# maxwellsh/DIGDriver

Measured on AMD Instinct MI355X. Metric: genomic elements tested/sec (whole node), whole-genome x 37 cohorts, higher is better.
Workload: dtype f64

## Files before the change

digdriver_amd/csrc/dig_nb.hip:

```cpp
#include <algorithm>
#include <cstdlib>

#include "dig_common.hpp"
#include "dig_math.hpp"

namespace dig {

constexpr int kBlock = 256;

struct OpMidpUpper {
    __device__ static double apply(double k, double a, double p) { return nb_midp_upper(k, a, p); }
};
struct OpExact {
    __device__ static double apply(double k, double a, double p) { return nb_exact(k, a, p); }
};
struct OpGreater {
    __device__ static double apply(double k, double a, double p) { return nb_greater(k, a, p); }
};
struct OpMidpTwo {
    __device__ static double apply(double k, double a, double p) { return nb_midp_twosided(k, a, p); }
};

template <typename Op>
__global__ __launch_bounds__(kBlock) void nb3_kernel(const double* __restrict__ k, const double* __restrict__ alpha,
// ... 96 lines not shown
    const int64_t e = a.use_fastdiv ? fastdiv(i, a.divC) : i;
    return load_raw(a, i, e, i - e * a.C);
}

__device__ __forceinline__ PairInputs prepare_pair(const PairRaw& w, bool has_indel_params)
{
    PairInputs r;
    r.k_snv = (double)w.k_snv;
    r.k_smp = (double)w.k_smp;
    r.k_ind = (double)w.k_ind;
    const GammaParams g = normal_params_to_gamma(w.mu, w.sigma);
    r.alpha = g.alpha;
    r.theta = mul_rn(g.theta, w.cj);
    r.exp_snv = mul_rn(mul_rn(g.alpha, r.theta), w.pi_s);
    r.p = nb_success_prob(r.theta, w.pi_s);
    GammaParams gi = g;
    if (has_indel_params) gi = normal_params_to_gamma(w.mu_i, w.sigma_i);
    r.alpha_i = gi.alpha;
    r.theta_i = mul_rn(gi.theta, w.cji);
    r.exp_ind = mul_rn(mul_rn(gi.alpha, r.theta_i), w.pi_i);
    r.p_i = nb_success_prob(r.theta_i, w.pi_i);
    return r;
}

__device__ __forceinline__ PairInputs load_pair(const ElementStatsArgs& a, int64_t i)
{
    return prepare_pair(load_raw(a, i), a.mu_indel != nullptr);
}

__global__ __launch_bounds__(kBlock) void element_stats_single_pass_kernel(ElementStatsArgs a)
{
    nb_tables_init();
    const int64_t n = a.E * a.C;
    const int64_t i = (int64_t)blockIdx.x * kBlock + threadIdx.x;
    if (i >= n) return;
    const PairInputs q = load_pair(a, i);
    double pv_snv = 0.0, pv_smp = 0.0, pv_ind = 0.0, dummy = 0.0;
    const unsigned d1 = nb_midp_upper_fast2(q.k_snv, q.k_smp, 3u, q.alpha, q.p, pv_snv, pv_smp);
    const unsigned d2 = nb_midp_upper_fast2(q.k_ind, 0.0, 1u, q.alpha_i, q.p_i, pv_ind, dummy);
    if (!(d1 & 1u)) pv_snv = nb_midp_upper_unresolved(q.k_snv, q.alpha, q.p);
    if (!(d1 & 2u)) pv_smp = nb_midp_upper_unresolved(q.k_smp, q.alpha, q.p);
    if (!(d2 & 1u)) pv_ind = nb_midp_upper_unresolved(q.k_ind, q.alpha_i, q.p_i);
    a.out[0 * n + i] = q.exp_snv;
    a.out[1 * n + i] = pv_snv;
    a.out[2 * n + i] = pv_smp;
    a.out[3 * n + i] = q.theta_i;
    a.out[4 * n + i] = q.exp_ind;
    a.out[5 * n + i] = pv_ind;
    a.out[6 * n + i] = fisher_combine_fast(pv_snv, pv_ind);
}

constexpr int kParkCap = 256;

__device__ __forceinline__ unsigned park_flush(unsigned* worklist, const unsigned* park, unsigned count, int lane)
{
    unsigned base = 0;
    if (lane == 0) base = atomicAdd(worklist, count);
    base = __shfl(base, 0, 64);
    for (unsigned j = lane; j < count; j += 64) worklist[kWorkHeader + base + j] = park[j];
    return 0;
}

#define DIG_STREAM_STORE(ptr, val) __builtin_nontemporal_store((val), (ptr))
template <bool HAS_INDEL_PARAMS, bool FUSED_RATES = false>
__global__ __launch_bounds__(kBlock) void element_stats_stream_kernel(ElementStatsArgs a)
{
    static_assert(!FUSED_RATES, "the rate sums are formed by element_stats_stream_fused_kernel");
    __shared__ unsigned park_all[kBlock / 64][kParkCap];
    nb_tables_init();
    unsigned* park = park_all[threadIdx.x >> 6];
    const int64_t n = a.E * a.C;
    const int lane = threadIdx.x & 63;
    const unsigned long long lanes_below = (1ull << lane) - 1ull;
    const int64_t n_tiles = (n + 63) >> 6;
    const int64_t n_waves = ((int64_t)gridDim.x * kBlock) >> 6;
    int64_t tile = ((int64_t)blockIdx.x * kBlock + threadIdx.x) >> 6;
    if (tile >= n_tiles) return;
    const int64_t step_pairs = n_waves * 64;
    const int64_t step_e = a.use_fastdiv ? fastdiv(step_pairs, a.divC) : step_pairs;
    const uint32_t step_c = (uint32_t)(step_pairs - step_e * a.C);
    const uint32_t C32 = (uint32_t)a.C;
    int64_t iu = tile * 64 + lane;
    int64_t eu = a.use_fastdiv ? fastdiv(iu, a.divC) : iu;
    uint32_t cu = (uint32_t)(iu - eu * a.C);
    auto clamped_load = [&]() {
        const bool past = iu >= n;
        return load_raw(a, past ? n - 1 : iu, past ? a.E - 1 : eu, past ? (int64_t)(C32 - 1) : (int64_t)cu);
    };
    PairRaw nxt = clamped_load();
    unsigned parked = 0;
    for (; tile < n_tiles; tile += n_waves) {
        if (parked > (unsigned)(kParkCap - 64)) parked = park_flush(a.worklist, park, parked, lane);
        const int64_t i_raw = tile * 64 + lane;
        const int64_t i = min(i_raw, n - 1);
        PairRaw cur = nxt;
        iu += step_pairs;
        eu += step_e;
        cu += step_c;
        if (cu >= C32) {
            cu -= C32;
            eu += 1;
        }
        nxt = clamped_load();
        const PairInputs q = prepare_pair(cur, HAS_INDEL_PARAMS);
        double pv_snv, pv_smp, pv_ind, dummy;
        const unsigned d1 = nb_fast2_counts<1>(cur.k_snv, cur.k_smp, true, q.alpha, q.p, pv_snv, pv_smp);
        const unsigned d2 = nb_fast2_counts<1>(cur.k_ind, 0, false, q.alpha_i, q.p_i, pv_ind, dummy);
        const bool slow = ((d1 != 3u) || (d2 != 1u)) && i_raw < n;
        const unsigned long long m = __ballot(slow);
        if (slow) park[parked + __popcll(m & lanes_below)] = (unsigned)i;
        parked += (unsigned)__popcll(m);
        DIG_STREAM_STORE(&a.out[0 * n + i], q.exp_snv);
        DIG_STREAM_STORE(&a.out[1 * n + i], pv_snv);
        DIG_STREAM_STORE(&a.out[2 * n + i], pv_smp);
        DIG_STREAM_STORE(&a.out[3 * n + i], q.theta_i);
        DIG_STREAM_STORE(&a.out[4 * n + i], q.exp_ind);
        DIG_STREAM_STORE(&a.out[5 * n + i], pv_ind);
        double pv_mut = 0.0;
        if (!slow) pv_mut = fisher_combine_fast(pv_snv, pv_ind);
        DIG_STREAM_STORE(&a.out[6 * n + i], pv_mut);
    }
    if (parked) park_flush(a.worklist, park, parked, lane);
}

constexpr int kPre = 2;

struct StagePtr {
    int64_t q0, q1;
    uint32_t i, e, c;
    uint32_t ok;
};
struct StageIn {
    int32_t idx[kPre];
    double mu, sg, mu_i, sg_i;
    double pi_s, pi_i, cj, cji;
    int k_snv, k_smp, k_ind;
    int64_t q0;
    uint32_t nb, i, c;
};
struct StageBin {
    double mu[kPre], sd[kPre];
    int32_t y[kPre];
    uint8_t fl[kPre];
};

constexpr int kQueueCap = 1024;
constexpr int kRecDoubles = 11;
__shared__ double g_queue[kQueueCap * kRecDoubles];
typedef double v2d __attribute__((ext_vector_type(2)));
__shared__ unsigned g_queue_list[16][48];
__shared__ unsigned g_queue_len, g_ovf_len, g_ovf_next;
__shared__ unsigned g_tests[3 * kQueueCap];
__shared__ unsigned g_n_tests, g_next_test;
constexpr int kSlowBlock = 256;
constexpr int kSlowWaves = kSlowBlock / 64;
constexpr int kSlowPairsPerWave = 8;
constexpr int kOverflowSlack = 64 * 1024;
__device__ __forceinline__ void slow_round(const ElementStatsArgs& a, const unsigned* __restrict__ items, unsigned base,
                                           unsigned count, bool have_first, unsigned first_item, double (*sp_all)[10],
                                           unsigned* list, int64_t n);

template <int TB, bool TICKETS, int GIVEN = 0, bool REC = false>
__global__ __launch_bounds__(TB) void element_stats_stream_fused_kernel(ElementStatsArgs a)
{
    static_assert(TB == 1024 && TICKETS, "one 1024-thread workgroup per CU drawing tile tickets");
    static_assert(!REC || GIVEN == 0 || GIVEN == 3, "record outputs: the pipeline's kernel only");
    double* const queue = g_queue;
    unsigned* const tests = g_tests;
    constexpr int QCAP = kQueueCap;
    constexpr bool FUSED = GIVEN == 0 || GIVEN == 3;
    constexpr bool PACKED = GIVEN == 3;
    __shared__ unsigned park_all[TB / 64][kParkCap];
    __shared__ unsigned s_ticket;
    if (threadIdx.x == 0) s_ticket = 0;
    if (threadIdx.x == 0) g_queue_len = g_ovf_len = g_ovf_next = g_n_tests = g_next_test = 0;
    nb_tables_init();
    unsigned* park = park_all[threadIdx.x >> 6];
    const int64_t n = a.E * a.C;
    const int lane = threadIdx.x & 63;
    const unsigned long long lanes_below = (1ull << lane) - 1ull;
    const int64_t n_tiles = (n + 63) >> 6;
    int64_t tile = ((int64_t)blockIdx.x * TB + threadIdx.x) >> 6;
    const uint32_t C32 = (uint32_t)a.C;
    int64_t iu = tile * 64 + lane;
    int64_t eu = a.use_fastdiv ? fastdiv(iu, a.divC) : iu;
    uint32_t cu = (uint32_t)(iu - eu * a.C);
    auto draw = [&]() -> int64_t {
        unsigned t = 0;
        if (lane == 0) t = atomicAdd(&s_ticket, 1u);
        t = (unsigned)__builtin_amdgcn_readfirstlane((int)t);
        if ((gridDim.x & 7u) == 0u) return ((int64_t)t * 8 + (blockIdx.x & 7u)) * (gridDim.x >> 3) + (blockIdx.x >> 3);
        return (int64_t)t * gridDim.x + blockIdx.x;
    };
    int64_t tile_ptr = 0;
    auto fetch_ptr = [&]() {
        StagePtr s;
        tile_ptr = draw();
        iu = tile_ptr * 64 + lane;
        eu = a.use_fastdiv ? fastdiv(min(iu, n - 1), a.divC) : iu;
        cu = (uint32_t)(min(iu, n - 1) - eu * a.C);
        const bool past = iu >= n;
        s.ok = (uint32_t)(tile_ptr < n_tiles);
        s.i = (uint32_t)(past ? n - 1 : iu);
        s.e = (uint32_t)(past ? a.E - 1 : eu);
        s.c = past ? C32 - 1 : cu;
        if (FUSED) {
            s.q0 = a.ov_ptr[s.e];
            s.q1 = a.ov_ptr[s.e + 1];
        } else
            s.q0 = s.q1 = 0;
        return s;
    };
    const int64_t nnz = FUSED ? a.ov_ptr[a.E] : 0;
    const int32_t* oi_base = nnz > 0 ? a.ov_idx : reinterpret_cast<const int32_t*>(a.ov_ptr);
    const int64_t oi_last = nnz > 0 ? nnz - 1 : 0;
    auto fetch_in = [&](const StagePtr& s) {
        StageIn r;
        r.q0 = s.q0;
        r.nb = (uint32_t)(s.q1 - s.q0);
        r.i = s.i;
        r.c = s.c;
        if (FUSED) {
#pragma unroll
            for (int j = 0; j < kPre; ++j)
                r.idx[j] = oi_base[min(s.q0 + j, oi_last)];
        } else {
            r.mu = a.mu[s.i];
            r.sg = a.sigma[s.i];
            if (GIVEN == 2) {
                r.mu_i = a.mu_indel[s.i];
                r.sg_i = a.sigma_indel[s.i];
            }
        }
        r.pi_s = __builtin_nontemporal_load(&a.pi_sum[s.i]);
        r.pi_i = a.pi_indel_per_cohort ? a.pi_indel[s.i] : a.pi_indel[s.e];
        r.k_snv = __builtin_nontemporal_load(&a.obs_snv[s.i]);
        r.k_smp = __builtin_nontemporal_load(&a.obs_samples[s.i]);
        r.k_ind = __builtin_nontemporal_load(&a.obs_indel[s.i]);
        r.cj = a.cj[s.c];
        r.cji = a.cj_indel[s.c];
        return r;
    };
    auto fetch_bin = [&](const StageIn& r) {
        StageBin b;
        if (!FUSED) return b;
#pragma unroll
        for (int j = 0; j < kPre; ++j) {
            const int64_t o = a.small_index ? (int64_t)(__umul24((uint32_t)r.idx[j], C32) + r.c)
                                            : (int64_t)r.idx[j] * a.C + r.c;
            if (PACKED) {
            const double2 mv = a.bin_pack[o];
            const int32_t yf = a.bin_yf[o];
            b.mu[j] = mv.x;
            b.sd[j] = mv.y;
            b.y[j] = yf & 0x7fffffff;
            b.fl[j] = (uint8_t)((uint32_t)yf >> 31);
            } else {
            b.mu[j] = a.bin_mu[o];
            b.sd[j] = a.bin_std[o];
            b.y[j] = a.bin_y[o];
            b.fl[j] = a.bin_flag[o];
            }
        }
        return b;
    };
    __syncthreads();
    StagePtr ptr_n = fetch_ptr();
    tile = tile_ptr;
    StageIn in_c = fetch_in(ptr_n);
    ptr_n = fetch_ptr();
    int64_t tile_n1 = tile_ptr;
    StageBin bin_c = fetch_bin(in_c);
    unsigned parked = 0;
    unsigned* segment = a.worklist + kWorkHeader + (int64_t)blockIdx.x * (((n_tiles + gridDim.x - 1) / gridDim.x) << 6);
    auto flush = [&](unsigned count) -> unsigned {
        unsigned base = 0;
        if (lane == 0) base = atomicAdd(&g_ovf_len, count);
        base = (unsigned)__builtin_amdgcn_readfirstlane((int)base);
        for (unsigned j = lane; j < count; j += 64) segment[base + j] = park[j];
        return 0;
    };
    for (; tile < n_tiles; tile = tile_n1) {
        if (parked > (unsigned)(kParkCap - 64)) parked = flush(parked);
        const bool live = tile * 64 + lane < n;
        const StageIn cur = in_c;
        const StageBin bin = bin_c;
        in_c = fetch_in(ptr_n);
        tile_n1 = tile_ptr;
        ptr_n = fetch_ptr();
        const int64_t i = cur.i;
        double mu = 0.0, var = 0.0;
        int robs = 0, flag = 0;
        if (FUSED) {
#pragma unroll
        for (int j = 0; j < kPre; ++j) {
            if ((uint32_t)j < cur.nb) {
                mu += bin.mu[j];
                var += PACKED ? bin.sd[j] : mul_rn(bin.sd[j], bin.sd[j]);
                robs += bin.y[j];
                flag |= (bin.fl[j] != 0);
            }
        }
        if (__any(cur.nb > (uint32_t)kPre)) {
            const int32_t* oi = a.ov_idx + cur.q0;
            for (uint32_t j = kPre; j < cur.nb; ++j) {
                const int64_t o = (int64_t)oi[j] * a.C + cur.c;
                if (PACKED) {
                    const double2 mv = a.bin_pack[o];
                    const int32_t yf = a.bin_yf[o];
                    mu += mv.x;
                    var += mv.y;
                    robs += yf & 0x7fffffff;
                    flag |= (int)((uint32_t)yf >> 31);
                } else {
                    const double sd = a.bin_std[o];
                    mu += a.bin_mu[o];
                    var += mul_rn(sd, sd);
                    robs += a.bin_y[o];
                    flag |= (a.bin_flag[o] != 0);
                }
            }
        }
        }
        PairRaw w;
        if (FUSED) {
            w.mu = w.mu_i = mu;
            w.sigma = w.sigma_i = sqrt(var);
        } else {
            w.mu = w.mu_i = cur.mu;
            w.sigma = w.sigma_i = cur.sg;
            if (GIVEN == 2) {
                w.mu_i = cur.mu_i;
                w.sigma_i = cur.sg_i;
            }
        }
        w.pi_s = cur.pi_s; w.pi_i = cur.pi_i; w.cj = cur.cj; w.cji = cur.cji;
        w.k_snv = cur.k_snv; w.k_smp = cur.k_smp; w.k_ind = cur.k_ind;
        w.c = cur.c;
        const PairInputs q = prepare_pair(w, GIVEN == 2);
        double pv_snv, pv_smp, pv_ind, dummy;
        const unsigned d1 = nb_fast2_counts<1>(w.k_snv, w.k_smp, true, q.alpha, q.p, pv_snv, pv_smp);
        const unsigned d2 = nb_fast2_counts<1>(w.k_ind, 0, false, q.alpha_i, q.p_i, pv_ind, dummy);
        const bool slow = ((d1 != 3u) || (d2 != 1u)) && live;
        double pv_mut = 0.0;
        if (!slow) pv_mut = fisher_combine_fast(pv_snv, pv_ind);
        bin_c = fetch_bin(in_c);
        unsigned long long m = __ballot(slow);
        if (m) {
            const unsigned cnt = (unsigned)__popcll(m);
            unsigned qb = 0;
            if (lane == 0) qb = atomicAdd(&g_queue_len, cnt);
            qb = (unsigned)__builtin_amdgcn_readfirstlane((int)qb);
            const unsigned slot = qb + (unsigned)__popcll(m & lanes_below);
            const bool fits = slot < (unsigned)QCAP;
            if (slow && fits) {
                double* r = queue + slot * kRecDoubles;
                r[0] = pv_snv; r[1] = pv_smp; r[2] = pv_ind;
                r[3] = q.k_snv; r[4] = q.k_smp; r[5] = q.k_ind;
                r[6] = q.alpha; r[7] = q.p; r[8] = q.alpha_i; r[9] = q.p_i;
                r[10] = __longlong_as_double((long long)i);
            }
            m = __ballot(slow && !fits);
        }
        if (slow && ((m >> lane) & 1ull)) park[parked + __popcll(m & lanes_below)] = (unsigned)i;
        parked += (unsigned)__popcll(m);
        if (REC) {
            const unsigned long long rf = (unsigned long long)(unsigned)robs | ((unsigned long long)(unsigned)flag << 32);
            v2d* g = reinterpret_cast<v2d*>(a.out + tile * (64 * kRecOut)) + lane;
#define DIG_REC_STORE(j, x, y) __builtin_nontemporal_store(v2d{(x), (y)}, &g[(j) * 64])
            DIG_REC_STORE(0, q.exp_snv, pv_snv);
            DIG_REC_STORE(1, pv_smp, q.theta_i);
            DIG_REC_STORE(2, q.exp_ind, pv_ind);
            DIG_REC_STORE(3, pv_mut, w.mu);
            DIG_REC_STORE(4, w.sigma, __longlong_as_double((long long)rf));
            continue;
        }
        if (FUSED) {
            DIG_STREAM_STORE(&a.mu_w[i], w.mu);
            DIG_STREAM_STORE(&a.sigma_w[i], w.sigma);
            DIG_STREAM_STORE(&a.r_obs[i], robs);
            DIG_STREAM_STORE(&a.flag[i], flag);
        }
        DIG_STREAM_STORE(&a.out[0 * n + i], q.exp_snv);
        DIG_STREAM_STORE(&a.out[1 * n + i], pv_snv);
        DIG_STREAM_STORE(&a.out[2 * n + i], pv_smp);
        DIG_STREAM_STORE(&a.out[3 * n + i], q.theta_i);
        DIG_STREAM_STORE(&a.out[4 * n + i], q.exp_ind);
        DIG_STREAM_STORE(&a.out[5 * n + i], pv_ind);
        DIG_STREAM_STORE(&a.out[6 * n + i], pv_mut);
    }
    if (parked) flush(parked);
    __syncthreads();
    const int total = (int)min(g_queue_len, (unsigned)QCAP);
    if (threadIdx.x == 0 && total) atomicAdd(&a.worklist[3], (unsigned)total);
    if (total) {
        const int rec = (int)threadIdx.x;
        double* r = queue + (rec < QCAP ? rec : 0) * kRecDoubles;
        unsigned open = 0;
        if (rec < total)
            open = (__double_as_longlong(r[0]) < 0 ? 1u : 0u) | (__double_as_longlong(r[1]) < 0 ? 2u : 0u) |
                   (__double_as_longlong(r[2]) < 0 ? 4u : 0u);
        const unsigned long long b0 = __ballot(open & 1u), b1 = __ballot(open & 2u), b2 = __ballot(open & 4u);
        const unsigned c0 = (unsigned)__popcll(b0), c1 = (unsigned)__popcll(b1), c2 = (unsigned)__popcll(b2);
        unsigned tb = 0;
        if (lane == 0 && c0 + c1 + c2) tb = atomicAdd(&g_n_tests, c0 + c1 + c2);
        tb = (unsigned)__builtin_amdgcn_readfirstlane((int)tb);
        if (open & 1u) tests[tb + (unsigned)__popcll(b0 & lanes_below)] = (unsigned)rec * 4u;
        if (open & 2u) tests[tb + c0 + (unsigned)__popcll(b1 & lanes_below)] = (unsigned)rec * 4u + 1u;
        if (open & 4u) tests[tb + c0 + c1 + (unsigned)__popcll(b2 & lanes_below)] = (unsigned)rec * 4u + 2u;
        __syncthreads();
        const unsigned n_tests = g_n_tests;
        const int quad = lane >> 2, sub = lane & 3;
        for (;;) {
            unsigned t0 = 0;
            if (lane == 0) t0 = atomicAdd(&g_next_test, 16u);
            t0 = (unsigned)__builtin_amdgcn_readfirstlane((int)t0);
            if (t0 >= n_tests) break;
            const bool active = t0 + (unsigned)quad < n_tests;
            const unsigned id = tests[active ? t0 + (unsigned)quad : t0];
            const int role = (int)(id & 3u);
            double* sp = queue + (id >> 2) * kRecDoubles;
            const double marker = sp[role];
            const double pv = nb_midp_upper_quad(sp[3 + role], sp[role == 2 ? 8 : 6], sp[role == 2 ? 9 : 7],
                                                 marker == -2.0 ? -1.0 : -marker, sub);
            if (active && sub == 0) sp[role] = pv;
        }
        __syncthreads();
        if (rec < total) {
            const int64_t item = __double_as_longlong(r[10]);
            const double pv_snv = r[0], pv_smp = r[1], pv_ind = r[2];
            if (REC) {
                a.out[rec_index(item, 1, n)] = pv_snv;
                a.out[rec_index(item, 2, n)] = pv_smp;
                a.out[rec_index(item, 5, n)] = pv_ind;
                a.out[rec_index(item, 6, n)] = fisher_combine_fast(pv_snv, pv_ind);
            } else {
                a.out[1 * n + item] = pv_snv;
                a.out[2 * n + item] = pv_smp;
                a.out[5 * n + item] = pv_ind;
                a.out[6 * n + item] = fisher_combine_fast(pv_snv, pv_ind);
            }
        }
    }
    const unsigned ovf = g_ovf_len;
    if (ovf) {
        __syncthreads();
        if (threadIdx.x == 0) atomicAdd(&a.worklist[2], ovf);
        double (*sp)[10] = reinterpret_cast<double (*)[10]>(queue + (threadIdx.x >> 6) * (kSlowPairsPerWave * 10));
        for (;;) {
            unsigned b = 0;
            if (lane == 0) b = atomicAdd(&g_ovf_next, (unsigned)kSlowPairsPerWave);
            b = (unsigned)__builtin_amdgcn_readfirstlane((int)b);
            if (b >= ovf) break;
            slow_round(a, segment, b, ovf, false, 0u, sp, g_queue_list[threadIdx.x >> 6], n);
        }
    }
}


__device__ __forceinline__ void slow_round(const ElementStatsArgs& a, const unsigned* __restrict__ items, unsigned base,
                                           unsigned count, bool have_first, unsigned first_item, double (*sp_all)[10],
                                           unsigned* list, int64_t n)
{
    const int lane = threadIdx.x & 63, quad = lane >> 2, sub = lane & 3;
    const bool owner = lane < kSlowPairsPerWave && base + lane < count;
    int64_t item = 0;
    unsigned open = 0;
    if (owner) {
        item = have_first ? first_item : items[base + lane];
        const double v1 = *out_slot(a, 1, n, item), v2 = *out_slot(a, 2, n, item), v5 = *out_slot(a, 5, n, item);
        const PairInputs q = load_pair(a, item);
        double* sp = sp_all[lane];
        sp[0] = v1; sp[1] = v2; sp[2] = v5;
        sp[3] = q.k_snv; sp[4] = q.k_smp; sp[5] = q.k_ind;
        sp[6] = q.alpha; sp[7] = q.p; sp[8] = q.alpha_i; sp[9] = q.p_i;
        open = (__double_as_longlong(v1) < 0 ? 1u : 0u) | (__double_as_longlong(v2) < 0 ? 2u : 0u) |
               (__double_as_longlong(v5) < 0 ? 4u : 0u);
    }
    const unsigned long long W = ((unsigned long long)__ballot(open & 1u) & 0xffffull) |
                                 (((unsigned long long)__ballot(open & 2u) & 0xffffull) << 16) |
                                 (((unsigned long long)__ballot(open & 4u) & 0xffffull) << 32);
    const int n_tests = __popcll(W);
    if (lane < 48 && ((W >> lane) & 1ull)) list[__popcll(W & ((1ull << lane) - 1ull))] = (unsigned)lane;
    __builtin_amdgcn_s_waitcnt(0xc07f);
    __builtin_amdgcn_wave_barrier();
    for (int t0 = 0; t0 < n_tests; t0 += 16) {
        const int t = t0 + quad;
        const bool active = t < n_tests;
        const unsigned bit = list[active ? t : 0];
        const int role = (int)(bit >> 4), slot = (int)(bit & 15u);
        const double* sp = sp_all[slot];
        const double marker = sp[role];
        const double k = sp[3 + role];
        const double al = sp[role == 2 ? 8 : 6], pp = sp[role == 2 ? 9 : 7];
        const double pv = nb_midp_upper_quad(k, al, pp, marker == -2.0 ? -1.0 : -marker, sub);
        if (active && sub == 0) sp_all[slot][role] = pv;
    }
    __builtin_amdgcn_s_waitcnt(0xc07f);
    __builtin_amdgcn_wave_barrier();
    if (owner) {
        const double* sp = sp_all[lane];
        const double pv_snv = sp[0], pv_smp = sp[1], pv_ind = sp[2];
        *out_slot(a, 1, n, item) = pv_snv;
        *out_slot(a, 2, n, item) = pv_smp;
        *out_slot(a, 5, n, item) = pv_ind;
        *out_slot(a, 6, n, item) = fisher_combine_fast(pv_snv, pv_ind);
    }
    __builtin_amdgcn_s_waitcnt(0xc07f);
    __builtin_amdgcn_wave_barrier();
}

__global__ __launch_bounds__(kSlowBlock) void element_stats_slow_kernel(ElementStatsArgs a)
{
    __shared__ double s_pair[kSlowWaves][kSlowPairsPerWave][10];
    __shared__ unsigned s_list[kSlowWaves][48];
    const int64_t n = a.E * a.C;
    const int tid = threadIdx.x, lane = tid & 63, wave = tid >> 6;
    const unsigned n_waves = gridDim.x * kSlowWaves;
    const unsigned base0 = (blockIdx.x * kSlowWaves + wave) * kSlowPairsPerWave;
    const unsigned count_raw = a.worklist[0];
    unsigned first_item = 0;
    if (lane < kSlowPairsPerWave && (int64_t)(base0 + lane) < n) first_item = a.worklist[kWorkHeader + base0 + lane];
    nb_tables_init();
    const unsigned count = (unsigned)min((int64_t)count_raw, n);
    if (blockIdx.x == 0 && tid == 0) a.worklist[2] = count;
    for (unsigned base = base0; base < count; base += n_waves * kSlowPairsPerWave)
        slow_round(a, a.worklist + kWorkHeader, base, count, base == base0, first_item, s_pair[wave], s_list[wave], n);
}

__global__ __launch_bounds__(kBlock) void tiled_nb_generic_kernel(const double* __restrict__ pt, int pt_per_cohort,
                                                                  const int32_t* __restrict__ k,
                                                                  const double* __restrict__ mu,
                                                                  const double* __restrict__ sigma,
                                                                  double* __restrict__ pval, double* __restrict__ exp_out,
                                                                  int64_t C, int64_t n_bins, int64_t n_tiles)
{
    nb_tables_init();
    const int64_t per_cohort = n_bins * n_tiles;
    const int64_t n = C * per_cohort;
    const int64_t stride = (int64_t)gridDim.x * kBlock;
    for (int64_t i = (int64_t)blockIdx.x * kBlock + threadIdx.x; i < n; i += stride) {
        const int64_t cb = i / n_tiles;
        const double m = mu[cb], s = sigma[cb];
        const double ptv = pt_per_cohort ? pt[i] : pt[i % per_cohort];
        const GammaParams g = normal_params_to_gamma(m, s);
        const double p = nb_success_prob(ptv, g.theta);
        pval[i] = nb_exact((double)k[i], g.alpha, p);
        exp_out[i] = mul_rn(ptv, m);
    }
}

constexpr int kTiledItems = 4;
constexpr int kTiledChunk = kBlock * kTiledItems;
constexpr int kTiledRowsMax = 64;

__global__ __launch_bounds__(kBlock) void tiled_nb_kernel(const double* __restrict__ pt, int pt_per_cohort,
                                                          const int32_t* __restrict__ k, const double* __restrict__ mu,
                                                          const double* __restrict__ sigma, double* __restrict__ pval,
                                                          double* __restrict__ exp_out, int64_t C, int64_t n_bins,
                                                          int64_t n_tiles, FastDiv div_tiles, FastDiv div_bins)
{
    __shared__ double s_alpha[kTiledRowsMax], s_theta[kTiledRowsMax], s_mu[kTiledRowsMax];
    nb_tables_init();
    const int64_t per_cohort = n_bins * n_tiles;
    const int64_t n = C * per_cohort;
    const int tid = threadIdx.x;
    for (int64_t chunk0 = (int64_t)blockIdx.x * kTiledChunk; chunk0 < n; chunk0 += (int64_t)gridDim.x * kTiledChunk) {
        const int64_t last = (chunk0 + kTiledChunk - 1 < n - 1) ? chunk0 + kTiledChunk - 1 : n - 1;
        const int64_t cb0 = fastdiv(chunk0, div_tiles);
        const int nrows = (int)(fastdiv(last, div_tiles) - cb0) + 1;
        if (tid < nrows) {
            const double m = mu[cb0 + tid];
            const GammaParams g = normal_params_to_gamma(m, sigma[cb0 + tid]);
            s_alpha[tid] = g.alpha;
            s_theta[tid] = g.theta;
            s_mu[tid] = m;
        }
        double ptv[kTiledItems];
        int kk[kTiledItems], row[kTiledItems];
#pragma unroll
        for (int u = 0; u < kTiledItems; ++u) {
            const int64_t i = chunk0 + u * kBlock + tid;
            const int64_t ic = i < n ? i : n - 1;
            const int64_t cb = fastdiv(ic, div_tiles);
            row[u] = (int)(cb - cb0);
            const int64_t c = n_bins > 1 ? fastdiv(cb, div_bins) : cb;
            ptv[u] = pt_per_cohort ? pt[ic] : pt[ic - c * per_cohort];
            kk[u] = k[ic];
        }
        __syncthreads();
#pragma unroll
        for (int u = 0; u < kTiledItems; ++u) {
            const int64_t i = chunk0 + u * kBlock + tid;
            if (i < n) {
                const double p = nb_success_prob(ptv[u], s_theta[row[u]]);
                __builtin_nontemporal_store(nb_exact((double)kk[u], s_alpha[row[u]], p), &pval[i]);
                __builtin_nontemporal_store(mul_rn(ptv[u], s_mu[row[u]]), &exp_out[i]);
            }
        }
        __syncthreads();
    }
}

template <typename Op>
static int launch_nb3(const double* k, const double* alpha, const double* p, double* out, int64_t n, void* stream)
{
    if (n == 0) return DIG_OK;
    if (!k || !alpha || !p || !out || n < 0) return set_error(DIG_EINVAL, "nb3: null pointer or negative n");
    hipLaunchKernelGGL(nb3_kernel<Op>, dim3(grid_for(n, kBlock)), dim3(kBlock), 0, (hipStream_t)stream, k, alpha, p,
                       out, n);
    DIG_HIP_TRY(hipGetLastError());
    return DIG_OK;
}

}

using namespace dig;

extern "C" {

int dig_nb_midp_upper(const double* k, const double* alpha, const double* p, double* out, int64_t n, void* stream)
{
    return launch_nb3<OpMidpUpper>(k, alpha, p, out, n, stream);
}
int dig_nb_exact(const double* k, const double* alpha, const double* p, double* out, int64_t n, void* stream)
{
    return launch_nb3<OpExact>(k, alpha, p, out, n, stream);
}
int dig_nb_greater(const double* k, const double* alpha, const double* p, double* out, int64_t n, void* stream)
{
    return launch_nb3<OpGreater>(k, alpha, p, out, n, stream);
}
int dig_nb_midp_twosided(const double* k, const double* alpha, const double* p, double* out, int64_t n, void* stream)
{
    return launch_nb3<OpMidpTwo>(k, alpha, p, out, n, stream);
}

int dig_fisher(const double* p1, const double* p2, double* out, int64_t n, void* stream)
{
    if (n == 0) return DIG_OK;
    DIG_REQUIRE(p1 && p2 && out && n > 0, "non-null pointers, n >= 0");
    hipLaunchKernelGGL(fisher_kernel, dim3(grid_for(n, kBlock)), dim3(kBlock), 0, (hipStream_t)stream, p1, p2, out, n);
    DIG_HIP_TRY(hipGetLastError());
    return DIG_OK;
}

int dig_normal_params_to_gamma(const double* mu, const double* sigma, double* alpha, double* theta, int64_t n,
                               void* stream)
{
    if (n == 0) return DIG_OK;
    DIG_REQUIRE(mu && sigma && alpha && theta && n > 0, "non-null pointers, n >= 0");
    hipLaunchKernelGGL(gamma_kernel, dim3(grid_for(n, kBlock)), dim3(kBlock), 0, (hipStream_t)stream, mu, sigma, alpha,
                       theta, n);
    DIG_HIP_TRY(hipGetLastError());
    return DIG_OK;
}

int64_t dig_element_stats_workspace(int64_t E, int64_t C)
{
    if (E < 0 || C < 0) return 0;
    const int64_t n = E * C;
    if (n >= (int64_t)0xffffffffu) return 0;
// ... 158 lines not shown
```

digdriver_amd/engine.py:

```python
import contextlib

import numpy as np

from . import _lib
from ._marshal import backend_of, backend_on, device_backend, is_cuda

ES_PLANES = _lib.ES_PLANES
GS_PLANES = _lib.GS_PLANES
SEL_PLANES = _lib.SEL_PLANES


def _t(x, dtype, device):
    return device_backend(device).arr(x, dtype)


_WS_CACHE = {}


def _workspace(kind, E, C, dev, private=False):
    import torch
    need = _lib.workspace_bytes(kind, E, C)
    if need <= 0:
        return None, 0
    if private:
        return torch.empty(need, dtype=torch.uint8, device=dev), need
    idx = dev.index if dev.index is not None else torch.cuda.current_device()
    key = (kind, idx, torch.cuda.current_stream(idx).cuda_stream)
    ws = _WS_CACHE.get(key)
    if ws is None or ws.numel() < need:
        ws = torch.empty(need, dtype=torch.uint8, device=dev)
        _WS_CACHE[key] = ws
    return ws, need


def _shared_workspace(be, kind, E, C, use=True):
    return _workspace(kind, E, C, be.dev) if be.is_device and use else (None, 0)


def _scan(be, counts, groups=None):
    n, g = counts.shape[0], 1 if groups is None else groups
    offsets, ends = be.empty(0, "i64"), np.zeros(g, np.int64)
    if n:
        incl = be.torch.cumsum(counts, 0, dtype=be.torch.int64) if be.is_device else np.cumsum(counts, dtype=np.int64)
        ends = incl[n // g - 1::n // g]
        offsets, ends = incl - counts, ends.cpu().numpy() if be.is_device else ends
    ptr = np.concatenate([[0], ends]).astype(np.int64)
    return (offsets, int(ptr[-1])) if groups is None else (offsets, int(ptr[-1]), ptr)


@contextlib.contextmanager
def _requirements_as_value_errors():
    try:
        yield
    except _lib.DigHipError as exc:
        if "requirement failed" in str(exc):
            raise ValueError(str(exc)) from exc
        raise


def _cols(a):
    return a[:, None] if a.ndim == 1 else a


def _per_cohort(be, x, C):
    x = be.arr(x, "f64", (-1,))
    if x is not None and x.shape[0] == 1 and C != 1:
        x = x.repeat(C)
    assert x is None or x.shape[0] == C
    return x


def _rates(be, mu, sigma, mu_indel, sigma_indel):
    mu = _cols(be.arr(mu, "f64"))
    n, C = mu.shape
    return mu, be.arr(sigma, "f64", (n, C)), be.arr(mu_indel, "f64", (n, C)), be.arr(sigma_indel, "f64", (n, C)), n, C


def element_stats(mu, sigma, pi_sum, pi_indel, obs_snv, obs_samples, obs_indel, cj, cj_indel,
                  mu_indel=None, sigma_indel=None, device=0, out=None, use_workspace=True):
    be = backend_of(mu, device=device)
    mu, sigma, mu_indel, sigma_indel, E, C = _rates(be, mu, sigma, mu_indel, sigma_indel)
    pi_sum = be.arr(pi_sum, "f64", (E, C))
    pi_indel = be.arr(pi_indel, "f64")
    per_cohort = int(pi_indel.ndim == 2)
    assert pi_indel.shape == ((E, C) if per_cohort else (E,))
    obs = [be.arr(v, "i32", (E, C)) for v in (obs_snv, obs_samples, obs_indel)]
    cj, cj_indel = _per_cohort(be, cj, C), _per_cohort(be, cj_indel, C)
    if out is None:
        out = be.empty((len(ES_PLANES), E, C), "f64")
    p = be.ptr
    be.call("dig_element_stats", p(mu), p(sigma), p(mu_indel), p(sigma_indel), p(pi_sum), p(pi_indel), per_cohort, p(obs[0]),
            p(obs[1]), p(obs[2]), p(cj), p(cj_indel), p(out), E, C,
            workspace=_shared_workspace(be, "element_stats", E, C, use_workspace))
    return {name: out[i] for i, name in enumerate(ES_PLANES)}


def _gene_observations(be, obs, n_samp, cj, t_indel, G, C):
    return be.arr(obs, "i32", (G, 5, C)), be.arr(n_samp, "i32", (G, 6, C)), _per_cohort(be, cj, C), _per_cohort(be, t_indel, C)


def gene_stats(mu, sigma, pi, pi_indel, obs, n_samp, cj, t_indel=None, mu_indel=None, sigma_indel=None, device=0, out=None):
    be = backend_of(mu, device=device)
    mu, sigma, mu_indel, sigma_indel, G, C = _rates(be, mu, sigma, mu_indel, sigma_indel)
    pi = be.arr(pi, "f64")
    if pi.ndim == 2:
        pi = pi[:, :, None]
    n_pi = pi.shape[1]
    assert pi.shape == (G, n_pi, C) and n_pi in (4, 6)
    pi_indel = be.arr(pi_indel, "f64")
    per_cohort = int(pi_indel is not None and pi_indel.ndim == 2)
    obs, n_samp, cj, ti = _gene_observations(be, obs, n_samp, cj, t_indel, G, C)
    if out is None:
        out = be.empty((len(GS_PLANES), G, C), "f64")
    p = be.ptr
    be.call("dig_gene_stats", p(mu), p(sigma), p(mu_indel), p(sigma_indel), p(pi), n_pi, p(pi_indel), per_cohort, p(obs), p(n_samp),
            p(cj), p(ti), int(ti is not None), p(out), G, C)
    return {name: out[i] for i, name in enumerate(GS_PLANES)}


def gene_selection(alpha, theta, pi, obs, device=0, out=None):
    be = backend_of(alpha, device=device)
    alpha = _cols(be.arr(alpha, "f64"))
    G, C = alpha.shape
    theta = be.arr(theta, "f64", (G, C))
    pi = be.arr(pi, "f64")
    if pi.ndim == 2:
        pi = pi[:, :, None]
    n_pi = pi.shape[1]
    assert pi.shape == (G, n_pi, C) and n_pi in (4, 6)
    obs = be.arr(obs, "i32", (G, 5, C))
    if out is None:
        out = be.empty((len(SEL_PLANES), G, C), "f64")
    p = be.ptr
    be.call("dig_gene_selection", p(alpha), p(theta), p(pi), n_pi, p(obs), p(out), G, C)
    return {name: out[i] for i, name in enumerate(SEL_PLANES)}


def join_blocks(chrom, start, end):
    chrom, start, end = (np.asarray(x, np.int64).ravel() for x in (chrom, start, end))
    order = np.lexsort((start, chrom))
    chrom, start, end_eff = chrom[order], start[order], np.where(end == start, start + 1, end)[order]
    runmax = np.empty_like(end_eff)
    for c in np.unique(chrom):
        sel = chrom == c
        runmax[sel] = np.maximum.accumulate(end_eff[sel])
    return order, (chrom << 40) | start, (chrom << 40) | runmax, end_eff


def _window_blocks(win_chrom, win_start, win_end):
    wc, ws, we = (np.asarray(x, np.int64).ravel() for x in (win_chrom, win_start, win_end))
    if len(wc) and (wc.min() < 0 or wc.max() >= (1 << 22) or ws.min() < 0 or max(ws.max(), we.max()) >= (1 << 40)):
        raise ValueError("windows: chromosome ids within [0, 2^22), coordinates within [0, 2^40)")
    return join_blocks(wc, ws, we)


def overlap_join(be, start_key, runmax_key, blk_end, m_chrom, m_start, m_end, max_pairs=None,
                 too_many="%d (row, block) pairs: more than max_pairs"):
    tabs = [be.arr(x, "i64", (-1,)) for x in (start_key, runmax_key, blk_end, m_chrom, m_start, m_end)]
    n_blk, n = tabs[0].shape[0], tabs[3].shape[0]
    assert tabs[1].shape[0] == tabs[2].shape[0] == n_blk and tabs[4].shape[0] == tabs[5].shape[0] == n
    if n == 0 or n_blk == 0:
        return be.empty(0, "i32"), be.empty(0, "i32")
    p = be.ptr
    join = [p(x) for x in tabs[:3]] + [n_blk] + [p(x) for x in tabs[3:]] + [n]
    counts = be.empty(n, "i32")
    be.call("dig_overlap_join_count", *join, p(counts))
    offsets, total = _scan(be, counts)
    if max_pairs is not None and total > max_pairs:
        raise ValueError(too_many % total)
    pair_row, pair_blk = be.empty(total, "i32"), be.empty(total, "i32")
    if total:
        be.call("dig_overlap_join_fill", *join, p(offsets), *([] if be.is_device else [total]), p(pair_row), p(pair_blk))
    return pair_row, pair_blk


def _sample_offsets(x, C=None):
    off = np.ascontiguousarray(np.asarray(x.cpu() if is_cuda(x) else x), dtype=np.int64).ravel()
    if (len(off) < 2 if C is None else len(off) != C + 1) or off[0] != 0 or (np.diff(off) < 0).any():
        raise ValueError("sample_offsets: C + 1 non-decreasing entries, 0 first")
    return off, len(off) - 1, int(off[-1])


def _sorted(be, keys):
    return keys.sort()[0] if be.is_device else np.sort(keys)

# ... 857 lines not shown
```

Before: 26.05 billion.

## Drain queued slow-path NB tests during the streaming loop instead of after barrier

Slow-path tail tests are now published into the shared test list as soon as records are queued, using unpublished sentinels and release fences. Waves can claim and evaluate batches of 16 tests inside the main tile loop through a CAS-based drain. This is meant to overlap the quad-precision NB tail work with streaming and shrink the serialized phase after the final barrier. It adds shared-memory atomics and a per-tile drain check to the hot loop, plus diagnostic counters written to the worklist header and a Python helper to read them.

```diff
diff --git a/digdriver_amd/csrc/dig_nb.hip b/digdriver_amd/csrc/dig_nb.hip
--- a/digdriver_amd/csrc/dig_nb.hip
+++ b/digdriver_amd/csrc/dig_nb.hip
@@ -272,13 +272,15 @@
 __shared__ unsigned g_queue_len, g_ovf_len, g_ovf_next;
 __shared__ unsigned g_tests[3 * kQueueCap];
 __shared__ unsigned g_n_tests, g_next_test;
+__shared__ unsigned g_inflight;
+constexpr unsigned kTestUnpublished = 0xffffffffu;
 constexpr int kSlowBlock = 256;
 constexpr int kSlowWaves = kSlowBlock / 64;
 constexpr int kSlowPairsPerWave = 8;
 constexpr int kOverflowSlack = 64 * 1024;
-__device__ __forceinline__ void slow_round(const ElementStatsArgs& a, const unsigned* __restrict__ items, unsigned base,
-                                           unsigned count, bool have_first, unsigned first_item, double (*sp_all)[10],
-                                           unsigned* list, int64_t n);
+__device__ __forceinline__ int slow_round(const ElementStatsArgs& a, const unsigned* __restrict__ items, unsigned base,
+                                          unsigned count, bool have_first, unsigned first_item, double (*sp_all)[10],
+                                          unsigned* list, int64_t n);
 
 template <int TB, bool TICKETS, int GIVEN = 0, bool REC = false>
 __global__ __launch_bounds__(TB) void element_stats_stream_fused_kernel(ElementStatsArgs a)
@@ -293,7 +295,8 @@
     __shared__ unsigned park_all[TB / 64][kParkCap];
     __shared__ unsigned s_ticket;
     if (threadIdx.x == 0) s_ticket = 0;
-    if (threadIdx.x == 0) g_queue_len = g_ovf_len = g_ovf_next = g_n_tests = g_next_test = 0;
+    if (threadIdx.x == 0) g_queue_len = g_ovf_len = g_ovf_next = g_n_tests = g_next_test = g_inflight = 0;
+    for (int j = (int)threadIdx.x; j < 3 * QCAP; j += TB) tests[j] = kTestUnpublished;
     nb_tables_init();
     unsigned* park = park_all[threadIdx.x >> 6];
     const int64_t n = a.E * a.C;
@@ -400,6 +403,32 @@
         for (unsigned j = lane; j < count; j += 64) segment[base + j] = park[j];
         return 0;
     };
+    auto drain = [&]() {
+        const unsigned have = (unsigned)__builtin_amdgcn_readfirstlane(
+            (int)__hip_atomic_load(&g_n_tests, __ATOMIC_RELAXED, __HIP_MEMORY_SCOPE_WORKGROUP));
+        const unsigned nt = (unsigned)__builtin_amdgcn_readfirstlane(
+            (int)__hip_atomic_load(&g_next_test, __ATOMIC_RELAXED, __HIP_MEMORY_SCOPE_WORKGROUP));
+        if (have < nt + 16u) return;
+        const unsigned id = __hip_atomic_load(&tests[nt + (unsigned)(lane >> 2)], __ATOMIC_RELAXED, __HIP_MEMORY_SCOPE_WORKGROUP);
+        if (__ballot(id == kTestUnpublished)) return;
+        unsigned won = 0;
+        if (lane == 0) {
+            unsigned expect = nt;
+            won = __hip_atomic_compare_exchange_strong(&g_next_test, &expect, nt + 16u, __ATOMIC_RELAXED, __ATOMIC_RELAXED,
+                                                       __HIP_MEMORY_SCOPE_WORKGROUP) ? 1u : 0u;
+        }
+        if (!__builtin_amdgcn_readfirstlane((int)won)) return;
+        __builtin_amdgcn_fence(__ATOMIC_ACQUIRE, "workgroup");
+        const int role = (int)(id & 3u);
+        int sub = lane & 3;
+        asm volatile("" : "+v"(sub));
+        double* sp = queue + (id >> 2) * kRecDoubles;
+        const double marker = sp[role];
+        const double pv = nb_midp_upper_quad(sp[3 + role], sp[role == 2 ? 8 : 6], sp[role == 2 ? 9 : 7],
+                                             marker == -2.0 ? -1.0 : -marker, sub);
+        if (sub == 0) sp[role] = pv;
+        if (lane == 0) atomicAdd(&g_inflight, 16u);
+    };
     for (; tile < n_tiles; tile = tile_n1) {
         if (parked > (unsigned)(kParkCap - 64)) parked = flush(parked);
         const bool live = tile * 64 + lane < n;
@@ -473,12 +502,32 @@
             qb = (unsigned)__builtin_amdgcn_readfirstlane((int)qb);
             const unsigned slot = qb + (unsigned)__popcll(m & lanes_below);
             const bool fits = slot < (unsigned)QCAP;
+            unsigned open = 0;
             if (slow && fits) {
                 double* r = queue + slot * kRecDoubles;
                 r[0] = pv_snv; r[1] = pv_smp; r[2] = pv_ind;
                 r[3] = q.k_snv; r[4] = q.k_smp; r[5] = q.k_ind;
                 r[6] = q.alpha; r[7] = q.p; r[8] = q.alpha_i; r[9] = q.p_i;
                 r[10] = __longlong_as_double((long long)i);
+                open = (__double_as_longlong(pv_snv) < 0 ? 1u : 0u) | (__double_as_longlong(pv_smp) < 0 ? 2u : 0u) |
+                       (__double_as_longlong(pv_ind) < 0 ? 4u : 0u);
+            }
+            const unsigned long long b0 = __ballot(open & 1u), b1 = __ballot(open & 2u), b2 = __ballot(open & 4u);
+            const unsigned c0 = (unsigned)__popcll(b0), c1 = (unsigned)__popcll(b1), c2 = (unsigned)__popcll(b2);
+            if (c0 + c1 + c2) {
+                unsigned tb = 0;
+                if (lane == 0) tb = atomicAdd(&g_n_tests, c0 + c1 + c2);
+                tb = (unsigned)__builtin_amdgcn_readfirstlane((int)tb);
+                __builtin_amdgcn_fence(__ATOMIC_RELEASE, "workgroup");
+                if (open & 1u)
+                    __hip_atomic_store(&tests[tb + (unsigned)__popcll(b0 & lanes_below)], slot * 4u, __ATOMIC_RELAXED,
+                                       __HIP_MEMORY_SCOPE_WORKGROUP);
+                if (open & 2u)
+                    __hip_atomic_store(&tests[tb + c0 + (unsigned)__popcll(b1 & lanes_below)], slot * 4u + 1u, __ATOMIC_RELAXED,
+                                       __HIP_MEMORY_SCOPE_WORKGROUP);
+                if (open & 4u)
+                    __hip_atomic_store(&tests[tb + c0 + c1 + (unsigned)__popcll(b2 & lanes_below)], slot * 4u + 2u, __ATOMIC_RELAXED,
+                                       __HIP_MEMORY_SCOPE_WORKGROUP);
             }
             m = __ballot(slow && !fits);
         }
@@ -493,6 +542,7 @@
             DIG_REC_STORE(2, q.exp_ind, pv_ind);
             DIG_REC_STORE(3, pv_mut, w.mu);
             DIG_REC_STORE(4, w.sigma, __longlong_as_double((long long)rf));
+            drain();
             continue;
         }
         if (FUSED) {
@@ -508,6 +558,7 @@
         DIG_STREAM_STORE(&a.out[4 * n + i], q.exp_ind);
         DIG_STREAM_STORE(&a.out[5 * n + i], pv_ind);
         DIG_STREAM_STORE(&a.out[6 * n + i], pv_mut);
+        drain();
     }
     if (parked) flush(parked);
     __syncthreads();
@@ -516,19 +567,6 @@
     if (total) {
         const int rec = (int)threadIdx.x;
         double* r = queue + (rec < QCAP ? rec : 0) * kRecDoubles;
-        unsigned open = 0;
-        if (rec < total)
-            open = (__double_as_longlong(r[0]) < 0 ? 1u : 0u) | (__double_as_longlong(r[1]) < 0 ? 2u : 0u) |
-                   (__double_as_longlong(r[2]) < 0 ? 4u : 0u);
-        const unsigned long long b0 = __ballot(open & 1u), b1 = __ballot(open & 2u), b2 = __ballot(open & 4u);
-        const unsigned c0 = (unsigned)__popcll(b0), c1 = (unsigned)__popcll(b1), c2 = (unsigned)__popcll(b2);
-        unsigned tb = 0;
-        if (lane == 0 && c0 + c1 + c2) tb = atomicAdd(&g_n_tests, c0 + c1 + c2);
-        tb = (unsigned)__builtin_amdgcn_readfirstlane((int)tb);
-        if (open & 1u) tests[tb + (unsigned)__popcll(b0 & lanes_below)] = (unsigned)rec * 4u;
-        if (open & 2u) tests[tb + c0 + (unsigned)__popcll(b1 & lanes_below)] = (unsigned)rec * 4u + 1u;
-        if (open & 4u) tests[tb + c0 + c1 + (unsigned)__popcll(b2 & lanes_below)] = (unsigned)rec * 4u + 2u;
-        __syncthreads();
         const unsigned n_tests = g_n_tests;
         const int quad = lane >> 2, sub = lane & 3;
         for (;;) {
@@ -545,6 +583,11 @@
                                                  marker == -2.0 ? -1.0 : -marker, sub);
             if (active && sub == 0) sp[role] = pv;
         }
+        if (threadIdx.x == 0 && n_tests) {
+            const unsigned early = g_inflight;
+            if (early) atomicAdd(&a.worklist[4], early);
+            if (n_tests - early) atomicAdd(&a.worklist[5], n_tests - early);
+        }
         __syncthreads();
         if (rec < total) {
             const int64_t item = __double_as_longlong(r[10]);
@@ -567,20 +610,22 @@
         __syncthreads();
         if (threadIdx.x == 0) atomicAdd(&a.worklist[2], ovf);
         double (*sp)[10] = reinterpret_cast<double (*)[10]>(queue + (threadIdx.x >> 6) * (kSlowPairsPerWave * 10));
+        unsigned late = 0;
         for (;;) {
             unsigned b = 0;
             if (lane == 0) b = atomicAdd(&g_ovf_next, (unsigned)kSlowPairsPerWave);
             b = (unsigned)__builtin_amdgcn_readfirstlane((int)b);
             if (b >= ovf) break;
-            slow_round(a, segment, b, ovf, false, 0u, sp, g_queue_list[threadIdx.x >> 6], n);
-        }
-    }
-}
-
-
-__device__ __forceinline__ void slow_round(const ElementStatsArgs& a, const unsigned* __restrict__ items, unsigned base,
-                                           unsigned count, bool have_first, unsigned first_item, double (*sp_all)[10],
-                                           unsigned* list, int64_t n)
+            late += (unsigned)slow_round(a, segment, b, ovf, false, 0u, sp, g_queue_list[threadIdx.x >> 6], n);
+        }
+        if (lane == 0 && late) atomicAdd(&a.worklist[5], late);
+    }
+}
+
+
+__device__ __forceinline__ int slow_round(const ElementStatsArgs& a, const unsigned* __restrict__ items, unsigned base,
+                                          unsigned count, bool have_first, unsigned first_item, double (*sp_all)[10],
+                                          unsigned* list, int64_t n)
 {
     const int lane = threadIdx.x & 63, quad = lane >> 2, sub = lane & 3;
     const bool owner = lane < kSlowPairsPerWave && base + lane < count;
@@ -628,6 +673,7 @@
     }
     __builtin_amdgcn_s_waitcnt(0xc07f);
     __builtin_amdgcn_wave_barrier();
+    return n_tests;
 }
 
 __global__ __launch_bounds__(kSlowBlock) void element_stats_slow_kernel(ElementStatsArgs a)
diff --git a/digdriver_amd/engine.py b/digdriver_amd/engine.py
--- a/digdriver_amd/engine.py
+++ b/digdriver_amd/engine.py
@@ -31,6 +31,16 @@
         ws = torch.empty(need, dtype=torch.uint8, device=dev)
         _WS_CACHE[key] = ws
     return ws, need
+
+
+def statistics_counters(kind, E, C, workspace=None, device=0):
+    import torch
+    dev = torch.device("cuda", device) if not isinstance(device, torch.device) else device
+    ws = workspace if workspace is not None else _workspace(kind, E, C, dev)[0]
+    off = 0 if kind == "element_stats" else (_lib.workspace_bytes("accumulate", E, C) + 255) // 256 * 256
+    torch.cuda.synchronize(dev)
+    h = ws[off:off + 24].view(torch.int32).cpu().tolist()
+    return {"pairs_overflow": h[2], "pairs_queue": h[3], "tests_in_flight": h[4], "tests_behind_barrier": h[5]}
 
 
 def _shared_workspace(be, kind, E, C, use=True):
```

Result: no change. 26.29 billion, median of 6 (+0.9%).
